# Wikinaut/agrep

Measured on NVIDIA H100. Metric: text_scan_throughput, higher is better.
Workload: dtype u32 bitwise

## Files before the change

agrep_b200/_lib.py:

```python
import ctypes as C
import os

HERE = os.path.dirname(os.path.abspath(__file__))
LIB_PATH = os.path.join(HERE, "libagrepb200.so")

AGB_MAXERR, AGB_MAXDELIM, AGB_MAXANCHOR = 8, 8, 24
WANT_COUNT, WANT_RECORDS, WANT_ORDINALS, WANT_LEVELS = 0, 1, 2, 4
PLAN_ALL, PLAN_ANCHORS = 0, 1
ENGINE_NAMES = {0: "bitap", 1: "asearch", 2: "asearch0", 3: "asearch1", 4: "sgrep_bm", 5: "regex"}
ENGINE_REGEX = 5
REGEX_MAXPOS = 63


class Options(C.Structure):
    _fields_ = [("k", C.c_int32), ("nocase", C.c_int32), ("wordbound", C.c_int32), ("wholeline", C.c_int32),
                ("inverse", C.c_int32), ("linenum", C.c_int32), ("ins_free", C.c_int32),
                ("cost_i", C.c_int32), ("cost_s", C.c_int32), ("cost_d", C.c_int32),
                ("bestmatch", C.c_int32), ("regex", C.c_int32), ("delim", C.c_char_p)]


class Desc(C.Structure):
    _fields_ = [("mask", C.c_uint64 * 256),
                ("init0", C.c_uint64), ("init1", C.c_uint64), ("noerr", C.c_uint64), ("endpos", C.c_uint64),
                ("dendpos", C.c_uint64), ("dmask", C.c_uint64), ("wildmask", C.c_uint64),
                ("reset", C.c_uint64 * (2 * AGB_MAXERR + 1)), ("start", C.c_uint64 * (2 * AGB_MAXERR + 1)),
                ("start_closes", C.c_int32), ("M", C.c_int32), ("L", C.c_int32),
                ("delim", C.c_uint8 * (2 * AGB_MAXDELIM + 2)),
                ("delim_kind", C.c_int32), ("k", C.c_int32), ("nrows", C.c_int32),
                ("cost_i", C.c_int32), ("cost_s", C.c_int32), ("cost_d", C.c_int32),
                ("engine", C.c_int32), ("and_mode", C.c_int32), ("inverse", C.c_int32),
                ("user_delim", C.c_int32), ("outtail", C.c_int32),
                ("plan", C.c_int32), ("n_anchors", C.c_int32), ("anchor_len", C.c_int32),
                ("anchor", C.c_uint32 * AGB_MAXANCHOR), ("anchor_fold", C.c_uint32), ("anchor_mask", C.c_uint32),
                ("refine", C.c_int32), ("pat_len", C.c_int32), ("anchor_off", C.c_int32 * AGB_MAXANCHOR),
                ("n_anchors3", C.c_int32), ("anchor3", C.c_uint32 * 4), ("anchor3_off", C.c_int32 * 4), ("adaptive", C.c_int32),
                ("delim_fold", C.c_uint8 * (2 * AGB_MAXDELIM + 2)), ("pad_", C.c_uint8 * 2)]


class Regex(C.Structure):
    _fields_ = [("follow", C.c_uint64 * (REGEX_MAXPOS + 1)), ("head", C.c_int32), ("tail", C.c_int32), ("pad", C.c_int32 * 2)]


class Record(C.Structure):
    _fields_ = [("begin", C.c_int64), ("end", C.c_int64), ("ordinal", C.c_int64), ("level", C.c_int32), ("pad", C.c_int32)]


class Result(C.Structure):
    _fields_ = [("n_matched", C.c_uint64), ("n_records", C.c_uint64), ("n_flagged", C.c_uint64),
                ("level_hist", C.c_uint64 * (AGB_MAXERR + 1)), ("ms_front", C.c_float), ("ms_records", C.c_float),
                ("n_closes", C.c_uint64), ("truncated", C.c_uint32), ("pad", C.c_uint32)]

# ... 82 lines not shown
```

agrep_b200/csrc/aux.cu:

```cuda
#include "automaton.cuh"
#include "corpus.h"

__global__ void __launch_bounds__(256) k_gram_sample(const uint8_t *text, uint64_t n_chunks, uint32_t nblk, uint32_t blk_chunks,
                                                    int ngram, const uint32_t *gram, const uint32_t *gmask, uint32_t fold, unsigned int *counts)
{
	__shared__ unsigned int s_cnt[128];
	if (threadIdx.x < 128) s_cnt[threadIdx.x] = 0;
	__syncthreads();
	const uint64_t t = (uint64_t)blockIdx.x * blockDim.x + threadIdx.x;
	const uint64_t b = t / blk_chunks, i = t % blk_chunks;
	if (b < nblk) {
		const uint64_t chunk = (n_chunks / nblk) * b + i;
		if (chunk + 2 < n_chunks) {
			const uint4 v = __ldg(reinterpret_cast<const uint4 *>(text) + chunk);
			const uint32_t x4 = __ldg(reinterpret_cast<const uint32_t *>(text) + (chunk + 1) * 4);
			const uint32_t x[5] = { v.x | fold, v.y | fold, v.z | fold, v.w | fold, x4 | fold };
			uint32_t wv[16];
#pragma unroll
			for (int w = 0; w < 4; w++) {
				wv[4 * w] = x[w]; wv[4 * w + 1] = __funnelshift_r(x[w], x[w + 1], 8);
				wv[4 * w + 2] = __funnelshift_r(x[w], x[w + 1], 16); wv[4 * w + 3] = __funnelshift_r(x[w], x[w + 1], 24);
			}
			for (int g = 0; g < ngram; g++) {
				const uint32_t G = gram[g], M = gmask[g];
				bool hit = false;
#pragma unroll
				for (int s = 0; s < 16; s++) hit = hit || ((wv[s] & M) == G);
				if (hit) atomicAdd(&s_cnt[g], 1u);
			}
		}
	}
	__syncthreads();
	if (threadIdx.x < ngram && s_cnt[threadIdx.x]) atomicAdd(&counts[threadIdx.x], s_cnt[threadIdx.x]);
}

__global__ void __launch_bounds__(256) k_bitmap_sample(const uint32_t *bitmap, uint64_t n_words, uint32_t stride, unsigned long long *out)
{
	unsigned long long c = 0;
	for (uint64_t i = ((uint64_t)blockIdx.x * blockDim.x + threadIdx.x) * stride; i < n_words; i += (uint64_t)gridDim.x * blockDim.x * stride)
		c += __popc(bitmap[i]);
	c = __reduce_add_sync(0xffffffffu, (uint32_t)c);
	if ((threadIdx.x & 31) == 0 && c) atomicAdd(out, c);
}

__global__ void __launch_bounds__(COMPACT_THREADS) k_compact_count(const uint32_t *bitmap, uint64_t n_words, uint32_t *block_counts, unsigned long long *totals)
{
	const uint64_t w0 = ((uint64_t)blockIdx.x * COMPACT_THREADS + threadIdx.x) * COMPACT_WPT;
	uint32_t c = 0;
// ... 361 lines not shown
```

agrep_b200/csrc/front.cu:

```cuda
#include "scan_internal.cuh"
#include "tma.cuh"


template <int NA, bool MASKED, bool POLY, int N3>
__device__ __forceinline__ uint32_t windows_test(uint32_t lo, uint32_t hi, const FrontParams &P, uint32_t acc)
{
	uint32_t w[4] = { lo, __funnelshift_r(lo, hi, 8), __funnelshift_r(lo, hi, 16), __funnelshift_r(lo, hi, 24) };
	if (POLY && N3 > 0) {
#pragma unroll
		for (int t = 0; t < 4; t++) {
			uint32_t r = (NA >= 2) ? __viaddmin_u32(w[t], P.coef[NA - 1], 0xFFFFFFFFu) : w[t] * P.one + P.coef[NA - 1];
#pragma unroll
			for (int i = NA - 2; i >= 0; i--) r = r * w[t] + P.coef[i];
			if (MASKED) r *= P.scale;
			uint32_t q;
			if (N3 == 1) q = w[t] * P.s256 + P.coef3[0];
			else {
				q = w[t] * P.one + P.coef3[N3 - 1];
#pragma unroll
				for (int i = N3 - 2; i >= 0; i--) q = q * w[t] + P.coef3[i];
				q *= P.s256;
			}
			acc = __vimin3_u32(acc, r, q);
		}
// ... 10 lines not shown
		}
		acc = __vimin3_u32(acc, f[0], f[1]);
		acc = __vimin3_u32(acc, f[2], f[3]);
	} else {
		if (MASKED) { w[0] &= P.amask; w[1] &= P.amask; w[2] &= P.amask; w[3] &= P.amask; }
#pragma unroll
		for (int a = 0; a < NA; a++) {
			uint32_t A = P.anchor[a];
			acc = __vimin3_u32(acc, w[0] - A, w[1] - A);
			acc = __vimin3_u32(acc, w[2] - A, w[3] - A);
		}
	}
	return acc;
}

template <int NA, bool MASKED, bool FOLD, bool POLY, bool FULL, bool COUNT, int N3>
__device__ __forceinline__ void front_chunks(const FrontParams &P, const uint8_t *st, uint32_t tid, uint32_t lane, uint32_t rem, uint32_t *bm, uint16_t *nlb)
{
#pragma unroll
	for (int c = 0; c < FRONT_CH; c++) {
		const uint32_t idx = c * FRONT_THREADS + tid;
		uint4 v = *reinterpret_cast<const uint4 *>(st + idx * 16);
		uint32_t x4 = *reinterpret_cast<const uint32_t *>(st + idx * 16 + 16);
		if (COUNT) {
			const uint32_t xs[4] = { v.x, v.y, v.z, v.w };
			uint32_t cn = 0;
#pragma unroll
			for (int w = 0; w < 4; w++) {
				const uint32_t t = (xs[w] | P.dfold4) ^ P.delim4;
				uint32_t z = ~(((t & 0x7F7F7F7Fu) + 0x7F7F7F7Fu) | t | 0x7F7F7F7Fu);
				if (!FULL) {
					const int64_t valid = ((int64_t)rem - (int64_t)idx) * 16 - (int64_t)(P.n_chunks * 16 - P.n) - 4 * w;
					if (valid <= 0) z = 0; else if (valid < 4) z &= (1u << (8 * (uint32_t)valid)) - 1u;
				}
				cn += __popc(z);
			}
			const uint32_t blk = __reduce_add_sync(0xffffffffu, cn);
			if (lane == 0 && (FULL || idx < rem)) nlb[c * (FRONT_THREADS / 32)] = (uint16_t)blk;
		}
		if (FOLD) { v.x |= P.fold; v.y |= P.fold; v.z |= P.fold; v.w |= P.fold; x4 |= P.fold; }
		uint32_t acc = 0xffffffffu;
		acc = windows_test<NA, MASKED, POLY, N3>(v.x, v.y, P, acc);
		acc = windows_test<NA, MASKED, POLY, N3>(v.y, v.z, P, acc);
		acc = windows_test<NA, MASKED, POLY, N3>(v.z, v.w, P, acc);
		acc = windows_test<NA, MASKED, POLY, N3>(v.w, x4, P, acc);
		if (FULL) {
			const uint32_t word = __ballot_sync(0xffffffffu, acc == 0);
			if (lane == 0) bm[c * (FRONT_THREADS / 32)] = word;
		} else {
			const bool flag = (idx < rem) && (acc == 0 || idx + 2 >= rem);
			const uint32_t word = __ballot_sync(0xffffffffu, flag);
			if (lane == 0 && idx < rem) bm[c * (FRONT_THREADS / 32)] = word;
		}
	}
}

template <int NA, bool MASKED, bool FOLD, bool POLY, bool COUNT, int N3>
__global__ void __launch_bounds__(FRONT_THREADS, FRONT_CTAS_PER_SM)
k_front(const FrontParams P)
{
	extern __shared__ __align__(128) uint8_t s_ring[];
	__shared__ uint64_t s_bar[FRONT_NST];
	const uint32_t tid = threadIdx.x, lane = tid & 31;
	if (tid == 0) {
		for (int i = 0; i < FRONT_NST; i++) mbar_init(&s_bar[i], 1);
		asm volatile("fence.mbarrier_init.release.cluster;" ::: "memory");
	}
	__syncthreads();
	auto issue = [&](uint64_t it) {
		const uint64_t sg = P.stage_begin + blockIdx.x + it * gridDim.x;
		if (sg >= P.stage_end) return;
		const uint32_t slot = (uint32_t)(it % FRONT_NST);
// ... 2 lines not shown
		mbar_expect_tx(&s_bar[slot], bytes);
		bulk_g2s(s_ring + slot * FRONT_SLOT_BYTES, P.text + off, bytes, &s_bar[slot]);
	};
	if (tid == 0) for (int i = 0; i < FRONT_NST; i++) issue(i);
	const uint32_t warp_in_cta = tid >> 5;
	for (uint32_t it = 0;; it++) {
		const uint64_t sg = P.stage_begin + blockIdx.x + (uint64_t)it * gridDim.x;
		if (sg >= P.stage_end) break;
		const uint32_t slot = it % FRONT_NST;
		mbar_wait(&s_bar[slot], (it / FRONT_NST) & 1u);
		const uint8_t *st = s_ring + slot * FRONT_SLOT_BYTES;
		const uint64_t left = P.n_chunks - sg * FRONT_STAGE_CHUNKS;
		const uint32_t rem = left > 0xFFFF0000ull ? 0xFFFF0000u : (uint32_t)left;
		uint32_t *bm = P.bitmap + sg * FRONT_WORDS_PER_STAGE + warp_in_cta;
		const bool full = left >= FRONT_STAGE_CHUNKS + 2;
		uint16_t *nlb = COUNT ? P.nl_blocks + sg * FRONT_WORDS_PER_STAGE + warp_in_cta : nullptr;
		if (full) front_chunks<NA, MASKED, FOLD, POLY, true, COUNT, N3>(P, st, tid, lane, rem, bm, nlb);
		else front_chunks<NA, MASKED, FOLD, POLY, false, COUNT, N3>(P, st, tid, lane, rem, bm, nlb);
		__syncthreads();
		if (tid == 0) issue((uint64_t)it + FRONT_NST);
	}
}

template <int NA, bool MASKED, bool FOLD, bool POLY, bool COUNT, int N3>
static void launch_front_cnt(const FrontParams &P, unsigned grid, cudaStream_t st)
{
	static bool configured[64] = {false};
	int dev = 0; cudaGetDevice(&dev);
	if (!configured[dev & 63]) {
		cudaFuncSetAttribute(k_front<NA, MASKED, FOLD, POLY, COUNT, N3>, cudaFuncAttributeMaxDynamicSharedMemorySize, FRONT_SMEM);
		configured[dev & 63] = true;
	}
	k_front<NA, MASKED, FOLD, POLY, COUNT, N3><<<grid, FRONT_THREADS, FRONT_SMEM, st>>>(P);
}
template <int NA, bool MASKED, bool FOLD, bool POLY, int N3>
static void launch_front_one(const FrontParams &P, unsigned grid, cudaStream_t st)
{
	if (P.nl_blocks) launch_front_cnt<NA, MASKED, FOLD, POLY, true, N3>(P, grid, st);
	else launch_front_cnt<NA, MASKED, FOLD, POLY, false, N3>(P, grid, st);
}
template <int NA, bool POLY>
static void launch_front_na(const FrontParams &P, bool masked, bool fold, unsigned grid, cudaStream_t st)
{
	if (masked) { if (fold) launch_front_one<NA, true, true, POLY, 0>(P, grid, st); else launch_front_one<NA, true, false, POLY, 0>(P, grid, st); }
	else        { if (fold) launch_front_one<NA, false, true, POLY, 0>(P, grid, st); else launch_front_one<NA, false, false, POLY, 0>(P, grid, st); }
}
template <int NA>
static void launch_front_mixed(const FrontParams &P, bool fold, unsigned grid, cudaStream_t st)
// ... 247 lines not shown
	F.stage_end = (word_end + FRONT_WORDS_PER_STAGE - 1) / FRONT_WORDS_PER_STAGE;
	F.fold = d.anchor_fold; F.amask = d.anchor_mask;
	F.nl_blocks = count_delims ? W.ord_blocks : nullptr; F.dfold4 = d.delim_fold[0] * 0x01010101u; F.delim4 = (d.delim[0] | d.delim_fold[0]) * 0x01010101u;
	const uint64_t stages = F.stage_end - F.stage_begin;
	unsigned grid = (unsigned)std::min<uint64_t>(stages, (uint64_t)W.sm_count * FRONT_CTAS_PER_SM);
	if (!grid) grid = 1;
	bool masked = d.anchor_mask != 0xFFFFFFFFu, fold = d.anchor_fold != 0;
	int na = 0;
	for (int i = 0; i < d.n_anchors; i++) {
		bool dup = false;
		for (int j = 0; j < na; j++) if (F.anchor[j] == d.anchor[i]) dup = true;
		if (!dup) F.anchor[na++] = d.anchor[i];
	}
	F.one = 1; F.scale = 1; F.s256 = 256;
	for (int i = d.anchor_len; i < 4; i++) F.scale <<= 8;
	bool poly = poly_setup(F.anchor, na, 8 * d.anchor_len, F.coef);
	if (d.n_anchors3 > 0) {
		int n3 = 0; uint32_t a3[4];
		for (int i = 0; i < d.n_anchors3; i++) {
			bool dup = false;
			for (int j = 0; j < n3; j++) if (a3[j] == d.anchor3[i]) dup = true;
			if (!dup) a3[n3++] = d.anchor3[i];
		}
		uint32_t c3[AGB_MAXANCHOR];
		const bool poly3 = poly_setup(a3, n3, 24, c3);
		if (!(poly && poly3)) { snprintf(g_err, sizeof g_err, "internal: mixed anchor plan without a polynomial form"); return AGB_ERR_ARG; }
		F.n3 = n3;
		for (int i = 0; i < n3; i++) F.coef3[i] = c3[i];
		if (n3 == 1) F.coef3[0] = 0u - 256u * a3[0];
		switch (na) {
// ... 46 lines not shown
```

agrep_b200/csrc/pattern.c:

```c
#include "agrep_b200.h"
#include "pattern_internal.h"
#include <stdio.h>
#include <stdlib.h>
#include <string.h>

#define WIDTH 64
#define FAIL(...) do { if (err && errlen) snprintf(err, errlen, __VA_ARGS__); return AGB_ERR_PATTERN; } while (0)

enum { S_HYPHEN = 129, S_NOCARE = 130, S_NNLINE = 131, S_WORDB = 133, S_LPAREN = 134, S_RPAREN = 135,
       S_LRANGE = 136, S_RRANGE = 137, S_LANGLE = 138, S_RANGLE = 139, S_NOT = 140, S_WILD = 141,
       S_ORSYM = 142, S_ORPAT = 143, S_ANDPAT = 144, S_STAR = 145 };

typedef struct {
	uint64_t cls[4];
	int is_sep;
	int prot;
	int wild;
	int lit;
	int part;
} pos_t;

typedef struct {
	pos_t p[WIDTH + 4];
	int n;
// ... 733 lines not shown
	return AGB_OK;
}

int agb_pattern_from_desc(const agb_desc *d, agb_pattern **out, char *err, size_t errlen)
{
	agb_pattern *p; int rc;
	if (err && errlen) err[0] = 0;
	if (!d || !out) return AGB_ERR_ARG;
	p = (agb_pattern *)calloc(1, sizeof *p);
	if (!p) return AGB_ERR_NOMEM;
	p->d = *d;
	if (p->d.plan != AGB_PLAN_ANCHORS || p->d.n_anchors < 1 || p->d.n_anchors > AGB_MAXANCHOR || p->d.anchor_len < 2 || p->d.anchor_len > 4) {
		p->d.plan = AGB_PLAN_ALL; p->d.n_anchors = 0; p->d.refine = 0;
	}
	if (p->d.n_anchors3 < 0 || p->d.n_anchors3 > 2 || p->d.plan != AGB_PLAN_ANCHORS) p->d.n_anchors3 = 0;
	rc = agbi_derive(&p->d, err, errlen);
	if (rc) { free(p); *out = NULL; return rc; }
	*out = p;
	return AGB_OK;
}

void agb_pattern_free(agb_pattern *p) { free(p); }
const agb_desc *agb_pattern_desc(const agb_pattern *p) { return p ? &p->d : NULL; }

void agb_fill_ordinals(const agb_pattern *p, const void *h_text, uint64_t n, agb_record *records, uint64_t n_records)
{
	const agb_desc *d = &p->d; const unsigned char *t = (const unsigned char *)h_text;
	const int L = d->L; uint64_t i = 0; long long j = 0, run = 0, q, taken = -(1ll << 60); unsigned char fd[2 * AGB_MAXDELIM + 2]; int z, head = 1;
	if (!n_records) return;
	folded_delim(d, fd);
// ... 30 lines not shown
```

agrep_b200/csrc/scan.cu:

```cuda
#include "scan_internal.cuh"
#include "corpus.h"
#include <unistd.h>
#include <fcntl.h>
#include <sys/stat.h>
#include <mutex>
#include <thread>

thread_local char g_err[512];
std::atomic<uint64_t> g_launches{0};

extern "C" const char *agb_last_error(void) { return g_err; }
extern "C" const char *agb_version(void) { return "agrep-b200 0.1 (sm_90a)"; }
extern "C" uint64_t agb_kernel_launches(void) { return g_launches.load(); }
static void win_release(int dev);
extern "C" void agb_shutdown(void)
{
	int cur = 0; cudaGetDevice(&cur);
	for (int dev = 0; dev < 64; dev++) {
		win_release(dev);
		std::lock_guard<std::mutex> lk(g_ws_mu[dev]);
		Workspace &W = g_ws[dev];
		if (!W.totals && !W.bitmap && !W.h2d_text) continue;
		if (cudaSetDevice(dev) != cudaSuccess) { cudaGetLastError(); continue; }
		cudaDeviceSynchronize();
// ... 210 lines not shown
	res->n_closes = (want & AGB_WANT_ORDINALS) ? W.h_totals[13] + (uint64_t)W.ord_virt : 0;
	return AGB_OK;
}

static int ordinals_prepare_blocks(const agb_desc &d, Workspace &W, uint64_t n, cudaStream_t st)
{
	int rc = ordinals_reserve(d, W, n); if (rc) return rc;
	const uint64_t n_words = ((n + 15) / 16 + 31) / 32;
	if (W.ord_blocks_cap > n_words) CUDA_TRY(cudaMemsetAsync(W.ord_blocks + n_words, 0, (W.ord_blocks_cap - n_words) * sizeof(uint16_t), st));
	return AGB_OK;
}

#define PLAN_MIN_BYTES   (256ull << 20)
#define PLAN_SAMPLE_BLK  64
#define PLAN_BLK_CHUNKS  4096
static int adaptive_plan(const agb_desc &d, Workspace &W, const void *d_text, uint64_t n, cudaStream_t st, agb_desc *out)
{
	*out = d;
	if (!d.adaptive || !front_usable(d) || !d.refine || d.n_anchors3 || n < PLAN_MIN_BYTES || d.pat_len < 4 || d.pat_len > 60) return AGB_OK;
	const int need = d.k + 1;
	if (need > 9) return AGB_OK;
	uint64_t key = 1469598103934665603ull;
	{
		const unsigned char *b = (const unsigned char *)&d;
		for (size_t i = 0; i < sizeof d; i++) { key ^= b[i]; key *= 1099511628211ull; }
		key ^= (uint64_t)(uintptr_t)d_text; key *= 1099511628211ull; key ^= n; key *= 1099511628211ull;
	}
	if (W.plan_valid && W.plan_key == key) { *out = W.plan_desc; return AGB_OK; }
	int lit[64]; bool pair_any = false;
	for (int j = 0; j < d.pat_len; j++) {
		const uint64_t bit = 1ull << (d.M - (d.L + 2 + j));
		int cnt = 0, c0 = -1, c1 = -1;
		for (int c = 0; c < 256; c++) if (d.mask[c] & bit) { if (cnt == 0) c0 = c; else if (cnt == 1) c1 = c; cnt++; }
		lit[j] = -1;
		if (cnt == 1 && c0 != '\n' && c0 < 0x80) lit[j] = c0;
		else if (cnt == 2 && (c0 ^ c1) == 0x20 && c1 < 0x80) { lit[j] = c0 | 0x20; pair_any = true; }
	}
	const uint32_t fold = pair_any ? 0x20202020u : 0u;
	struct Gram { int s, len; uint32_t v, m; double cost; };
	Gram g[128]; int ng = 0;
	for (int len = 4; len >= 3; len--)
		for (int s = 0; s + len <= d.pat_len && ng < 120; s++) {
			bool ok = true; uint32_t v = 0;
			for (int t = 0; t < len; t++) { if (lit[s + t] < 0) ok = false; else v |= (uint32_t)(lit[s + t] | (fold & 0x20)) << (8 * t); }
			if (!ok) continue;
			g[ng].s = s; g[ng].len = len; g[ng].v = v; g[ng].m = len == 4 ? 0xFFFFFFFFu : 0x00FFFFFFu; g[ng].cost = 0; ng++;
		}
	if (ng < need) return AGB_OK;
	if (!W.d_gram) { CUDA_TRY(cudaMalloc(&W.d_gram, 3 * 128 * sizeof(uint32_t))); CUDA_TRY(cudaMallocHost(&W.h_gram, 3 * 128 * sizeof(uint32_t))); }
	for (int i = 0; i < 128; i++) { W.h_gram[i] = i < ng ? g[i].v : 0; W.h_gram[128 + i] = i < ng ? g[i].m : 0; W.h_gram[256 + i] = 0; }
	CUDA_TRY(cudaMemcpyAsync(W.d_gram, W.h_gram, 3 * 128 * sizeof(uint32_t), cudaMemcpyHostToDevice, st));
	const uint64_t n_chunks = (n + 15) / 16;
	const uint64_t threads = (uint64_t)PLAN_SAMPLE_BLK * PLAN_BLK_CHUNKS;
	k_gram_sample<<<(unsigned)((threads + 255) / 256), 256, 0, st>>>((const uint8_t *)d_text, n_chunks, PLAN_SAMPLE_BLK, PLAN_BLK_CHUNKS,
	                                                                 ng, W.d_gram, W.d_gram + 128, fold, W.d_gram + 256);
	g_launches++;
	CUDA_TRY(cudaGetLastError());
	CUDA_TRY(cudaMemcpyAsync(W.h_gram + 256, W.d_gram + 256, 128 * sizeof(uint32_t), cudaMemcpyDeviceToHost, st));
	CUDA_TRY(cudaStreamSynchronize(st));
	for (int i = 0; i < ng; i++) g[i].cost = (double)W.h_gram[256 + i] / (double)threads;
	const char *mp = getenv("AGB_PLAN_MIXED");
	const double INF = 1e30, MIXED = mp ? atof(mp) : 0.03;
	static double f[66][10][3]; static int from[66][10][3];
	for (int p = 0; p <= d.pat_len; p++) for (int j = 0; j <= need; j++) for (int t = 0; t < 3; t++) { f[p][j][t] = INF; from[p][j][t] = -2; }
	f[0][0][0] = 0;
	for (int p = 0; p < d.pat_len; p++)
		for (int j = 0; j <= need; j++) for (int t = 0; t < 3; t++) {
			if (f[p][j][t] >= INF) continue;
			if (f[p][j][t] < f[p + 1][j][t]) { f[p + 1][j][t] = f[p][j][t]; from[p + 1][j][t] = -1; }
			if (j == need) continue;
			for (int i = 0; i < ng; i++) if (g[i].s == p) {
				const int t2 = t + (g[i].len == 3), p2 = p + g[i].len;
				if (t2 > 2) continue;
				if (f[p][j][t] + g[i].cost < f[p2][j + 1][t2]) { f[p2][j + 1][t2] = f[p][j][t] + g[i].cost; from[p2][j + 1][t2] = i; }
			}
		}
	int best_t = -1; double best = INF;
	for (int t = 0; t < 3; t++) {
		if (need - t < 1 || need - t > (t ? 7 : 9)) continue;
		const double c = f[d.pat_len][need][t] + (t ? MIXED : 0);
		if (c < best) { best = c; best_t = t; }
	}
	double cur = 0;
	for (int a = 0; a < d.n_anchors; a++) { double r = 1.0; for (int i = 0; i < ng; i++) if (g[i].len == d.anchor_len && g[i].s == d.anchor_off[a]) r = g[i].cost; cur += r; }
	if (best_t < 0 || !(best < 0.85 * cur)) { W.plan_key = key; W.plan_valid = true; W.plan_desc = d; return AGB_OK; }
	agb_desc nd = d;
	nd.n_anchors = 0; nd.n_anchors3 = 0; nd.anchor_len = 4; nd.anchor_mask = 0xFFFFFFFFu; nd.anchor_fold = fold;
	{
		int p = d.pat_len, j = need, t = best_t;
		while (p > 0 && j >= 0) {
			const int fr = from[p][j][t];
			if (fr == -1) { p--; continue; }
			if (fr < 0) break;
			if (g[fr].len == 4) { nd.anchor[nd.n_anchors] = g[fr].v; nd.anchor_off[nd.n_anchors] = g[fr].s; nd.n_anchors++; }
			else { nd.anchor3[nd.n_anchors3] = g[fr].v; nd.anchor3_off[nd.n_anchors3] = g[fr].s; nd.n_anchors3++; }
			p -= g[fr].len; j--; t -= (g[fr].len == 3);
		}
	}
	bool ok = nd.n_anchors + nd.n_anchors3 == need && nd.n_anchors >= 1;
	uint32_t tmp[AGB_MAXANCHOR];
	if (ok) ok = poly_setup(nd.anchor, nd.n_anchors, 32, tmp);
	if (ok && nd.n_anchors3) ok = poly_setup(nd.anchor3, nd.n_anchors3, 24, tmp);
	for (int a = 0; a < nd.n_anchors && ok; a++) {
		for (int b = 0; b < a; b++) if (nd.anchor[a] == nd.anchor[b]) ok = false;
		for (int b = 0; b < nd.n_anchors3; b++) if ((nd.anchor[a] & 0x00FFFFFFu) == nd.anchor3[b]) ok = false;
	}
	for (int a = 0; a < nd.n_anchors3 && ok; a++) for (int b = 0; b < a; b++) if (nd.anchor3[a] == nd.anchor3[b]) ok = false;
	W.plan_key = key; W.plan_valid = true; W.plan_desc = ok ? nd : d;
	*out = W.plan_desc;
	if (getenv("AGB_DEBUG_PLAN")) {
		fprintf(stderr, "agb plan: static rate %.4f -> %s rate %.4f:", cur, ok ? "chosen" : "rejected", best);
		for (int a = 0; a < nd.n_anchors; a++) fprintf(stderr, " [%.4s]@%d", (const char *)&nd.anchor[a], nd.anchor_off[a]);
		for (int a = 0; a < nd.n_anchors3; a++) fprintf(stderr, " [%.3s]@%d", (const char *)&nd.anchor3[a], nd.anchor3_off[a]);
		fprintf(stderr, "\n");
	}
	return AGB_OK;
}

int shard_aux_enqueue(const agb_desc &d, Workspace &W, const uint8_t *text, uint64_t n, const ShardInfo *sh, bool ordinals, cudaStream_t st);

static int stages_after_front(const agb_desc &d, Workspace &W, const void *d_text, uint64_t n, bool use_front, bool count_in_front,
                              int want, int want_level, agb_record *d_records, uint64_t capacity, cudaStream_t st, agb_result *res,
                              const ShardInfo *sh = nullptr)
{
	int rc;
	const uint64_t n_chunks = (n + 15) / 16;
	if (use_front && refine_cannot_thin(d)) { bool dense = false; rc = front_is_dense(W, n, st, &dense); if (rc) return rc; if (dense) use_front = false; }
	bool refined = false;
	if (use_front) { rc = refine_launch(d, W, d_text, n, st, &refined); if (rc) return rc; }
	for (int attempt = 0; ; attempt++) {
// ... 34 lines not shown
		agb_result r;
		int rc = scan_device_impl(pos, d_text, n, AGB_WANT_COUNT | AGB_WANT_ORDINALS, -1, nullptr, 0, st, &r, nullptr); if (rc) return rc;
		unsigned char last = 0;
		CUDA_TRY(cudaMemcpyAsync(&last, (const uint8_t *)d_text + n - 1, 1, cudaMemcpyDeviceToHost, st));
		CUDA_TRY(cudaStreamSynchronize(st));
		const uint64_t records = r.n_closes - 2 + (last != '\n' ? 1 : 0);
		if (r.n_closes < 2 || r.n_matched > records) { snprintf(g_err, sizeof g_err, "internal: complement count out of range"); return AGB_ERR_CUDA; }
		*res = r;
		res->n_matched = records - r.n_matched; res->n_closes = 0; res->n_records = 0;
		return AGB_OK;
	}
	std::lock_guard<std::mutex> lk(g_ws_mu[dev]);
	Workspace &W = g_ws[dev];
	int rc = ws_prepare(W, n); if (rc) return rc;
	agb_desc planned;
	rc = adaptive_plan(d_in, W, d_text, n, st, &planned); if (rc) return rc;
	const agb_desc &d = planned;
	if (want == AGB_WANT_COUNT && !sh && n >= (1u << 20) && exact_count_usable(d)) {
		CUDA_TRY(cudaMemsetAsync(W.totals, 0, 16 * sizeof(unsigned long long), st));
		CUDA_TRY(cudaEventRecord(W.e0, st));
		rc = exact_count_launch(d, W, d_text, n, st); if (rc) return rc;
		CUDA_TRY(cudaEventRecord(W.e1, st));
		CUDA_TRY(cudaEventRecord(W.e2, st));
		rc = fetch_result(W, want, capacity, false, st, res); if (rc) return rc;
		res->n_flagged = 0;
		CUDA_TRY(cudaEventElapsedTime(&res->ms_front, W.e0, W.e1));
		res->ms_records = 0;
		return AGB_OK;
	}
	rc = ws_upload_desc(W, d, st); if (rc) return rc;
	rc = regex_prepare(W, d, rx, st); if (rc) return rc;
// ... 603 lines not shown
```

agrep_b200/csrc/scan_internal.cuh:

```cuda
#ifndef AGB_SCAN_INTERNAL_CUH
#define AGB_SCAN_INTERNAL_CUH
#include "agrep_b200.h"
#include "pattern_internal.h"
#include <cuda_runtime.h>
#include <stdint.h>
#include <stdio.h>
#include <string.h>
#include <stdlib.h>
#include <atomic>
#include <algorithm>

extern thread_local char g_err[512];
extern std::atomic<uint64_t> g_launches;

#define CUDA_TRY(x) do { cudaError_t e_ = (x); if (e_ != cudaSuccess) { \
	snprintf(g_err, sizeof g_err, "%s failed: %s (%s:%d)", #x, cudaGetErrorString(e_), __FILE__, __LINE__); \
	return AGB_ERR_CUDA; } } while (0)

#define FRONT_THREADS 256
#define FRONT_CH      4
#define FRONT_STAGE_CHUNKS (FRONT_THREADS * FRONT_CH)
#define FRONT_STAGE_BYTES  (FRONT_STAGE_CHUNKS * 16)
#define FRONT_SLOT_BYTES   (FRONT_STAGE_BYTES + 16)
#define FRONT_NST     2
// ... 140 lines not shown
int  exact_count_launch(const agb_desc &d, Workspace &W, const void *d_text, uint64_t n, cudaStream_t st);
bool poly_setup(const uint32_t *a, int na, int bits, uint32_t *coef);
int  front_launch(const agb_desc &d, Workspace &W, const void *d_text, uint64_t n, uint64_t word_begin, uint64_t word_end, bool slack16, cudaStream_t st, bool count_delims = false);
int  refine_launch(const agb_desc &d, Workspace &W, const void *d_text, uint64_t n, cudaStream_t st, bool *ran);
unsigned refine_grid(const Workspace &W, uint64_t n);
int  compact_ranges_launch(Workspace &W, uint64_t n, cudaStream_t st);
#define REFINE_MAX_RANGES 16384
int  launch_records(const agb_desc &d, const RecParams &P, unsigned grid, cudaStream_t st);
int  launch_dense(const agb_desc &d, const RecParams &P, unsigned grid, cudaStream_t st);
int  launch_records_list(const agb_desc &d, const RecParams &P, unsigned grid, cudaStream_t st);
int  launch_slices(const agb_desc &d, const RecParams &P, unsigned grid, cudaStream_t st);
bool slices_usable(const agb_desc &d);
int  launch_regex(const agb_desc &d, const RecParams &P, unsigned grid, cudaStream_t st);
size_t regex_tables(const agb_desc &d, const agb_regex &rx, uint64_t *out);
__global__ void k_gram_sample(const uint8_t *text, uint64_t n_chunks, uint32_t nblk, uint32_t blk_chunks,
                              int ngram, const uint32_t *gram, const uint32_t *gmask, uint32_t fold, unsigned int *counts);
__global__ void k_compact_count(const uint32_t *bitmap, uint64_t n_words, uint32_t *block_counts, unsigned long long *totals);
__global__ void k_compact_write(const uint32_t *bitmap, uint64_t n_words, const uint64_t *block_offsets, uint64_t *cand, uint64_t cand_cap);
__global__ void k_scan_tiles(const uint32_t *counts, uint64_t *offsets, uint64_t n_tiles, unsigned long long *total);
__global__ void k_scan_partial(const uint32_t *counts, uint64_t n, uint32_t *block_sums, const unsigned long long *n_dev);
__global__ void k_scan_apply(const uint32_t *counts, uint64_t n, const uint64_t *block_offsets, uint64_t *offsets, const unsigned long long *n_dev);
int  front_is_dense(Workspace &W, uint64_t n, cudaStream_t st, bool *dense);
int  ordinals_launch(const agb_desc &d, Workspace &W, const void *d_text, uint64_t n, agb_record *d_records, uint64_t capacity, cudaStream_t st, bool blocks_counted = false);
int  ordinals_reserve(const agb_desc &d, Workspace &W, uint64_t n);
#endif
```

include/agrep_b200.h:

```cpp
#ifndef AGREP_B200_H
#define AGREP_B200_H
#include <stdint.h>
#include <stddef.h>

#ifdef __cplusplus
extern "C" {
#endif

#define AGB_MAXERR    8
#define AGB_MAXDELIM  8
#define AGB_MAXANCHOR 24

enum {
	AGB_OK = 0,
	AGB_ERR_PATTERN = -1,
	AGB_ERR_CUDA = -2,
	AGB_ERR_ARG = -3,
	AGB_ERR_NOMEM = -4
};

typedef struct agb_options {
	int32_t k;
	int32_t nocase;
	int32_t wordbound;
// ... 30 lines not shown
	int32_t  nrows;
	int32_t  cost_i, cost_s, cost_d;
	int32_t  engine, and_mode, inverse, user_delim, outtail;
	int32_t  plan;
	int32_t  n_anchors, anchor_len;
	uint32_t anchor[AGB_MAXANCHOR];
	uint32_t anchor_fold;
	uint32_t anchor_mask;
	int32_t  refine, pat_len;
	int32_t  anchor_off[AGB_MAXANCHOR];
	int32_t  n_anchors3;
	uint32_t anchor3[4];
	int32_t  anchor3_off[4];
	int32_t  adaptive;
	uint8_t  delim_fold[2 * AGB_MAXDELIM + 2];
	uint8_t  pad_[2];
} agb_desc;

typedef struct agb_pattern agb_pattern;

#define AGB_REGEX_MAXPOS 63
typedef struct agb_regex {
	uint64_t follow[AGB_REGEX_MAXPOS + 1];
	int32_t  head, tail;
	int32_t  pad[2];
} agb_regex;

typedef struct agb_record {
	int64_t begin;
	int64_t end;
	int64_t ordinal;
// ... 95 lines not shown
```

Before: 2081.

## Add pair-of-pieces anchor filter plan chosen by adaptive sampling

Adds a new candidate-filter plan that splits the pattern into k+2 disjoint literal pieces and flags a chunk only when at least two distinct pieces occur within it or the adjacent chunk. The sampler now also measures the rate of this pair condition, and the planner picks it when that rate is well below the k+1 anchor plan's rate and delimiter counting for ordinals is not needed. The goal is fewer false-positive candidates reaching the costlier verification stage. In exchange the front kernel does per-piece presence checks with warp shuffles, and the sampling kernel does a second window load on hits.

Measured after the change: 2311, median of 6. 11.1% higher.

```diff
diff --git a/agrep_b200/_lib.py b/agrep_b200/_lib.py
--- a/agrep_b200/_lib.py
+++ b/agrep_b200/_lib.py
@@ -34,7 +34,7 @@
                 ("anchor", C.c_uint32 * AGB_MAXANCHOR), ("anchor_fold", C.c_uint32), ("anchor_mask", C.c_uint32),
                 ("refine", C.c_int32), ("pat_len", C.c_int32), ("anchor_off", C.c_int32 * AGB_MAXANCHOR),
                 ("n_anchors3", C.c_int32), ("anchor3", C.c_uint32 * 4), ("anchor3_off", C.c_int32 * 4), ("adaptive", C.c_int32),
-                ("delim_fold", C.c_uint8 * (2 * AGB_MAXDELIM + 2)), ("pad_", C.c_uint8 * 2)]
+                ("delim_fold", C.c_uint8 * (2 * AGB_MAXDELIM + 2)), ("pair_plan", C.c_uint8), ("pad_", C.c_uint8)]
 
 
 class Regex(C.Structure):
diff --git a/agrep_b200/csrc/aux.cu b/agrep_b200/csrc/aux.cu
--- a/agrep_b200/csrc/aux.cu
+++ b/agrep_b200/csrc/aux.cu
@@ -1,8 +1,27 @@
 #include "automaton.cuh"
 #include "corpus.h"
 
+__device__ __forceinline__ void sample_windows(const uint8_t *text, uint64_t chunk, uint32_t fold, uint32_t (&wv)[16])
+{
+	const uint4 v = __ldg(reinterpret_cast<const uint4 *>(text) + chunk);
+	const uint32_t x4 = __ldg(reinterpret_cast<const uint32_t *>(text) + (chunk + 1) * 4);
+	const uint32_t x[5] = { v.x | fold, v.y | fold, v.z | fold, v.w | fold, x4 | fold };
+#pragma unroll
+	for (int w = 0; w < 4; w++) {
+		wv[4 * w] = x[w]; wv[4 * w + 1] = __funnelshift_r(x[w], x[w + 1], 8);
+		wv[4 * w + 2] = __funnelshift_r(x[w], x[w + 1], 16); wv[4 * w + 3] = __funnelshift_r(x[w], x[w + 1], 24);
+	}
+}
+__device__ __forceinline__ bool sample_hit(const uint32_t (&wv)[16], uint32_t G, uint32_t M)
+{
+	bool hit = false;
+#pragma unroll
+	for (int s = 0; s < 16; s++) hit = hit || ((wv[s] & M) == G);
+	return hit;
+}
 __global__ void __launch_bounds__(256) k_gram_sample(const uint8_t *text, uint64_t n_chunks, uint32_t nblk, uint32_t blk_chunks,
-                                                    int ngram, const uint32_t *gram, const uint32_t *gmask, uint32_t fold, unsigned int *counts)
+                                                    int ngram, const uint32_t *gram, const uint32_t *gmask, uint32_t fold, unsigned int *counts,
+                                                    int pair_first, int n_pair)
 {
 	__shared__ unsigned int s_cnt[128];
 	if (threadIdx.x < 128) s_cnt[threadIdx.x] = 0;
@@ -12,26 +31,24 @@
 	if (b < nblk) {
 		const uint64_t chunk = (n_chunks / nblk) * b + i;
 		if (chunk + 2 < n_chunks) {
-			const uint4 v = __ldg(reinterpret_cast<const uint4 *>(text) + chunk);
-			const uint32_t x4 = __ldg(reinterpret_cast<const uint32_t *>(text) + (chunk + 1) * 4);
-			const uint32_t x[5] = { v.x | fold, v.y | fold, v.z | fold, v.w | fold, x4 | fold };
 			uint32_t wv[16];
-#pragma unroll
-			for (int w = 0; w < 4; w++) {
-				wv[4 * w] = x[w]; wv[4 * w + 1] = __funnelshift_r(x[w], x[w + 1], 8);
-				wv[4 * w + 2] = __funnelshift_r(x[w], x[w + 1], 16); wv[4 * w + 3] = __funnelshift_r(x[w], x[w + 1], 24);
+			sample_windows(text, chunk, fold, wv);
+			uint32_t here = 0;
+			for (int g = 0; g < ngram; g++) {
+				if (!sample_hit(wv, gram[g], gmask[g])) continue;
+				if (g < 127) atomicAdd(&s_cnt[g], 1u);
+				if (g >= pair_first && g < pair_first + n_pair) here |= 1u << (g - pair_first);
 			}
-			for (int g = 0; g < ngram; g++) {
-				const uint32_t G = gram[g], M = gmask[g];
-				bool hit = false;
-#pragma unroll
-				for (int s = 0; s < 16; s++) hit = hit || ((wv[s] & M) == G);
-				if (hit) atomicAdd(&s_cnt[g], 1u);
+			if (here) {
+				uint32_t next = 0;
+				sample_windows(text, chunk + 1, fold, wv);
+				for (int p = 0; p < n_pair; p++) if (sample_hit(wv, gram[pair_first + p], gmask[pair_first + p])) next |= 1u << p;
+				if (__popc(here | next) >= 2) atomicAdd(&s_cnt[127], 1u);
 			}
 		}
 	}
 	__syncthreads();
-	if (threadIdx.x < ngram && s_cnt[threadIdx.x]) atomicAdd(&counts[threadIdx.x], s_cnt[threadIdx.x]);
+	if (threadIdx.x < 128 && s_cnt[threadIdx.x]) atomicAdd(&counts[threadIdx.x], s_cnt[threadIdx.x]);
 }
 
 __global__ void __launch_bounds__(256) k_bitmap_sample(const uint32_t *bitmap, uint64_t n_words, uint32_t stride, unsigned long long *out)
diff --git a/agrep_b200/csrc/front.cu b/agrep_b200/csrc/front.cu
--- a/agrep_b200/csrc/front.cu
+++ b/agrep_b200/csrc/front.cu
@@ -48,6 +48,24 @@
 	return acc;
 }
 
+template <bool FULL>
+__device__ __forceinline__ uint32_t chunk_delims(const FrontParams &P, const uint4 v, uint32_t idx, uint32_t rem)
+{
+	const uint32_t xs[4] = { v.x, v.y, v.z, v.w };
+	uint32_t cn = 0;
+#pragma unroll
+	for (int w = 0; w < 4; w++) {
+		const uint32_t t = (xs[w] | P.dfold4) ^ P.delim4;
+		uint32_t z = ~(((t & 0x7F7F7F7Fu) + 0x7F7F7F7Fu) | t | 0x7F7F7F7Fu);
+		if (!FULL) {
+			const int64_t valid = ((int64_t)rem - (int64_t)idx) * 16 - (int64_t)(P.n_chunks * 16 - P.n) - 4 * w;
+			if (valid <= 0) z = 0; else if (valid < 4) z &= (1u << (8 * (uint32_t)valid)) - 1u;
+		}
+		cn += __popc(z);
+	}
+	return cn;
+}
+
 template <int NA, bool MASKED, bool FOLD, bool POLY, bool FULL, bool COUNT, int N3>
 __device__ __forceinline__ void front_chunks(const FrontParams &P, const uint8_t *st, uint32_t tid, uint32_t lane, uint32_t rem, uint32_t *bm, uint16_t *nlb)
 {
@@ -57,19 +75,7 @@
 		uint4 v = *reinterpret_cast<const uint4 *>(st + idx * 16);
 		uint32_t x4 = *reinterpret_cast<const uint32_t *>(st + idx * 16 + 16);
 		if (COUNT) {
-			const uint32_t xs[4] = { v.x, v.y, v.z, v.w };
-			uint32_t cn = 0;
-#pragma unroll
-			for (int w = 0; w < 4; w++) {
-				const uint32_t t = (xs[w] | P.dfold4) ^ P.delim4;
-				uint32_t z = ~(((t & 0x7F7F7F7Fu) + 0x7F7F7F7Fu) | t | 0x7F7F7F7Fu);
-				if (!FULL) {
-					const int64_t valid = ((int64_t)rem - (int64_t)idx) * 16 - (int64_t)(P.n_chunks * 16 - P.n) - 4 * w;
-					if (valid <= 0) z = 0; else if (valid < 4) z &= (1u << (8 * (uint32_t)valid)) - 1u;
-				}
-				cn += __popc(z);
-			}
-			const uint32_t blk = __reduce_add_sync(0xffffffffu, cn);
+			const uint32_t blk = __reduce_add_sync(0xffffffffu, chunk_delims<FULL>(P, v, idx, rem));
 			if (lane == 0 && (FULL || idx < rem)) nlb[c * (FRONT_THREADS / 32)] = (uint16_t)blk;
 		}
 		if (FOLD) { v.x |= P.fold; v.y |= P.fold; v.z |= P.fold; v.w |= P.fold; x4 |= P.fold; }
@@ -89,7 +95,68 @@
 	}
 }
 
-template <int NA, bool MASKED, bool FOLD, bool POLY, bool COUNT, int N3>
+
+__device__ __forceinline__ uint32_t imad(uint32_t a, uint32_t b, uint32_t c)
+{
+	uint32_t r; asm("mad.lo.u32 %0, %1, %2, %3;" : "=r"(r) : "r"(a), "r"(b), "r"(c)); return r;
+}
+
+template <int NP>
+__device__ __forceinline__ uint32_t piece_bits(const uint32_t (&x)[5], const FrontParams &P)
+{
+	uint32_t acc[NP];
+#pragma unroll
+	for (int i = 0; i < NP; i++) acc[i] = 1u;
+#pragma unroll
+	for (int w = 0; w < 4; w++) {
+		const uint32_t wv[4] = { x[w], __funnelshift_r(x[w], x[w + 1], 8), __funnelshift_r(x[w], x[w + 1], 16), __funnelshift_r(x[w], x[w + 1], 24) };
+#pragma unroll
+		for (int i = 0; i < NP; i++) {
+			acc[i] = __vimin3_u32(acc[i], imad(wv[0], P.scale, P.coef[i]), imad(wv[1], P.scale, P.coef[i]));
+			acc[i] = __vimin3_u32(acc[i], imad(wv[2], P.scale, P.coef[i]), imad(wv[3], P.scale, P.coef[i]));
+		}
+	}
+	uint32_t absent = 0;
+#pragma unroll
+	for (int i = 0; i < NP; i++) absent |= acc[i] << i;
+	return absent ^ ((1u << NP) - 1u);
+}
+
+template <int NP, bool FOLD, bool FULL, bool COUNT>
+__device__ __forceinline__ void pair_chunks(const FrontParams &P, const uint8_t *st, uint32_t wid, uint32_t lane, uint32_t rem, uint32_t *bm, uint16_t *nlb)
+{
+	uint32_t pres[FRONT_CH];
+#pragma unroll
+	for (int c = 0; c < FRONT_CH; c++) {
+		const uint32_t idx = (wid * FRONT_CH + c) * 32 + lane;
+		const uint4 v = *reinterpret_cast<const uint4 *>(st + idx * 16);
+		const uint32_t x4 = *reinterpret_cast<const uint32_t *>(st + idx * 16 + 16);
+		if (COUNT) {
+			const uint32_t blk = __reduce_add_sync(0xffffffffu, chunk_delims<FULL>(P, v, idx, rem));
+			if (lane == 0 && (FULL || idx < rem)) nlb[c] = (uint16_t)blk;
+		}
+		const uint32_t f = FOLD ? P.fold : 0u;
+		const uint32_t x[5] = { v.x | f, v.y | f, v.z | f, v.w | f, x4 | f };
+		pres[c] = piece_bits<NP>(x, P);
+	}
+#pragma unroll
+	for (int c = 0; c < FRONT_CH; c++) {
+		const uint32_t idx = (wid * FRONT_CH + c) * 32 + lane;
+		const uint32_t give = (lane == 0 && c + 1 < FRONT_CH) ? pres[c + 1] : pres[c];
+		uint32_t next = __shfl_sync(0xffffffffu, give, (lane + 1) & 31);
+		if (c + 1 == FRONT_CH && lane == 31) next = ~0u;
+		const bool pair = pres[c] != 0 && __popc(pres[c] | next) >= 2;
+		if (FULL) {
+			const uint32_t word = __ballot_sync(0xffffffffu, pair);
+			if (lane == 0) bm[c] = word;
+		} else {
+			const uint32_t word = __ballot_sync(0xffffffffu, (idx < rem) && (pair || idx + 2 >= rem));
+			if (lane == 0 && idx < rem) bm[c] = word;
+		}
+	}
+}
+
+template <int NA, bool MASKED, bool FOLD, bool POLY, bool COUNT, int N3, int NP = 0>
 __global__ void __launch_bounds__(FRONT_THREADS, FRONT_CTAS_PER_SM)
 k_front(const FrontParams P)
 {
@@ -122,24 +189,37 @@
 		const uint32_t rem = left > 0xFFFF0000ull ? 0xFFFF0000u : (uint32_t)left;
 		uint32_t *bm = P.bitmap + sg * FRONT_WORDS_PER_STAGE + warp_in_cta;
 		const bool full = left >= FRONT_STAGE_CHUNKS + 2;
-		uint16_t *nlb = COUNT ? P.nl_blocks + sg * FRONT_WORDS_PER_STAGE + warp_in_cta : nullptr;
-		if (full) front_chunks<NA, MASKED, FOLD, POLY, true, COUNT, N3>(P, st, tid, lane, rem, bm, nlb);
-		else front_chunks<NA, MASKED, FOLD, POLY, false, COUNT, N3>(P, st, tid, lane, rem, bm, nlb);
+		if constexpr (NP > 0) {
+			uint32_t *bmp = P.bitmap + sg * FRONT_WORDS_PER_STAGE + warp_in_cta * FRONT_CH;
+			uint16_t *nlp = COUNT ? P.nl_blocks + sg * FRONT_WORDS_PER_STAGE + warp_in_cta * FRONT_CH : nullptr;
+			if (full) pair_chunks<NP, FOLD, true, COUNT>(P, st, warp_in_cta, lane, rem, bmp, nlp);
+			else pair_chunks<NP, FOLD, false, COUNT>(P, st, warp_in_cta, lane, rem, bmp, nlp);
+		} else {
+			uint16_t *nlb = COUNT ? P.nl_blocks + sg * FRONT_WORDS_PER_STAGE + warp_in_cta : nullptr;
+			if (full) front_chunks<NA, MASKED, FOLD, POLY, true, COUNT, N3>(P, st, tid, lane, rem, bm, nlb);
+			else front_chunks<NA, MASKED, FOLD, POLY, false, COUNT, N3>(P, st, tid, lane, rem, bm, nlb);
+		}
 		__syncthreads();
 		if (tid == 0) issue((uint64_t)it + FRONT_NST);
 	}
 }
 
-template <int NA, bool MASKED, bool FOLD, bool POLY, bool COUNT, int N3>
+template <int NA, bool MASKED, bool FOLD, bool POLY, bool COUNT, int N3, int NP = 0>
 static void launch_front_cnt(const FrontParams &P, unsigned grid, cudaStream_t st)
 {
 	static bool configured[64] = {false};
 	int dev = 0; cudaGetDevice(&dev);
 	if (!configured[dev & 63]) {
-		cudaFuncSetAttribute(k_front<NA, MASKED, FOLD, POLY, COUNT, N3>, cudaFuncAttributeMaxDynamicSharedMemorySize, FRONT_SMEM);
+		cudaFuncSetAttribute(k_front<NA, MASKED, FOLD, POLY, COUNT, N3, NP>, cudaFuncAttributeMaxDynamicSharedMemorySize, FRONT_SMEM);
 		configured[dev & 63] = true;
 	}
-	k_front<NA, MASKED, FOLD, POLY, COUNT, N3><<<grid, FRONT_THREADS, FRONT_SMEM, st>>>(P);
+	k_front<NA, MASKED, FOLD, POLY, COUNT, N3, NP><<<grid, FRONT_THREADS, FRONT_SMEM, st>>>(P);
+}
+template <int NP>
+static void launch_front_pairs(const FrontParams &P, bool fold, unsigned grid, cudaStream_t st)
+{
+	if (P.nl_blocks) { if (fold) launch_front_cnt<0, false, true, true, true, 0, NP>(P, grid, st); else launch_front_cnt<0, false, false, true, true, 0, NP>(P, grid, st); }
+	else             { if (fold) launch_front_cnt<0, false, true, true, false, 0, NP>(P, grid, st); else launch_front_cnt<0, false, false, true, false, 0, NP>(P, grid, st); }
 }
 template <int NA, bool MASKED, bool FOLD, bool POLY, int N3>
 static void launch_front_one(const FrontParams &P, unsigned grid, cudaStream_t st)
@@ -417,6 +497,18 @@
 	}
 	F.one = 1; F.scale = 1; F.s256 = 256;
 	for (int i = d.anchor_len; i < 4; i++) F.scale <<= 8;
+	if (d.pair_plan) {
+		if (na != d.n_anchors || na < 2 || na > 4 || d.anchor_len < 3) { snprintf(g_err, sizeof g_err, "internal: pair plan with %d pieces", d.n_anchors); return AGB_ERR_ARG; }
+		for (int i = 0; i < na; i++) F.coef[i] = 0u - F.anchor[i] * F.scale;
+		switch (na) {
+		case 2: launch_front_pairs<2>(F, fold, grid, st); break;
+		case 3: launch_front_pairs<3>(F, fold, grid, st); break;
+		default: launch_front_pairs<4>(F, fold, grid, st); break;
+		}
+		g_launches++;
+		CUDA_TRY(cudaGetLastError());
+		return AGB_OK;
+	}
 	bool poly = poly_setup(F.anchor, na, 8 * d.anchor_len, F.coef);
 	if (d.n_anchors3 > 0) {
 		int n3 = 0; uint32_t a3[4];
diff --git a/agrep_b200/csrc/pattern.c b/agrep_b200/csrc/pattern.c
--- a/agrep_b200/csrc/pattern.c
+++ b/agrep_b200/csrc/pattern.c
@@ -771,6 +771,7 @@
 		p->d.plan = AGB_PLAN_ALL; p->d.n_anchors = 0; p->d.refine = 0;
 	}
 	if (p->d.n_anchors3 < 0 || p->d.n_anchors3 > 2 || p->d.plan != AGB_PLAN_ANCHORS) p->d.n_anchors3 = 0;
+	p->d.pair_plan = 0;
 	rc = agbi_derive(&p->d, err, errlen);
 	if (rc) { free(p); *out = NULL; return rc; }
 	*out = p;
diff --git a/agrep_b200/csrc/scan.cu b/agrep_b200/csrc/scan.cu
--- a/agrep_b200/csrc/scan.cu
+++ b/agrep_b200/csrc/scan.cu
@@ -248,17 +248,45 @@
 #define PLAN_MIN_BYTES   (256ull << 20)
 #define PLAN_SAMPLE_BLK  64
 #define PLAN_BLK_CHUNKS  4096
-static int adaptive_plan(const agb_desc &d, Workspace &W, const void *d_text, uint64_t n, cudaStream_t st, agb_desc *out)
+#define PAIR_REACH       16
+
+static int pair_pieces(const int *lit, int pat_len, int k, uint32_t fold, uint32_t *val, int *off, int *len_out)
+{
+	const int np = k + 2;
+	if (k < 0 || np > 4) return 0;
+	for (int len = 4; len >= 3; len--)
+		for (int s0 = 0; s0 + np * len <= pat_len; s0++) {
+			int got = 0;
+			for (int p = s0; p + len <= pat_len && got < np; ) {
+				bool ok = true; uint32_t v = 0;
+				for (int t = 0; t < len; t++) { if (lit[p + t] < 0) ok = false; else v |= (uint32_t)(lit[p + t] | (fold & 0x20)) << (8 * t); }
+				if (!ok) { p++; continue; }
+				val[got] = v; off[got] = p; got++; p += len;
+			}
+			if (got < np || off[0] != s0 || off[np - 1] - off[0] + k > PAIR_REACH) continue;
+			bool distinct = true;
+			for (int a = 0; a < np; a++) for (int b = 0; b < a; b++) if (val[a] == val[b]) distinct = false;
+			if (!distinct) continue;
+			*len_out = len;
+			return np;
+		}
+	return 0;
+}
+
+static int adaptive_plan(const agb_desc &d, Workspace &W, const void *d_text, uint64_t n, bool count_delims, cudaStream_t st, agb_desc *out)
 {
 	*out = d;
 	if (!d.adaptive || !front_usable(d) || !d.refine || d.n_anchors3 || n < PLAN_MIN_BYTES || d.pat_len < 4 || d.pat_len > 60) return AGB_OK;
 	const int need = d.k + 1;
 	if (need > 9) return AGB_OK;
+	const char *pp = getenv("AGB_PLAN_PAIRS");
+	const int pairs_env = (pp && *pp) ? atoi(pp) : -1;
 	uint64_t key = 1469598103934665603ull;
 	{
 		const unsigned char *b = (const unsigned char *)&d;
 		for (size_t i = 0; i < sizeof d; i++) { key ^= b[i]; key *= 1099511628211ull; }
 		key ^= (uint64_t)(uintptr_t)d_text; key *= 1099511628211ull; key ^= n; key *= 1099511628211ull;
+		key ^= (uint64_t)(pairs_env + 2) * 2 + (count_delims ? 1 : 0); key *= 1099511628211ull;
 	}
 	if (W.plan_valid && W.plan_key == key) { *out = W.plan_desc; return AGB_OK; }
 	int lit[64]; bool pair_any = false;
@@ -280,19 +308,27 @@
 			if (!ok) continue;
 			g[ng].s = s; g[ng].len = len; g[ng].v = v; g[ng].m = len == 4 ? 0xFFFFFFFFu : 0x00FFFFFFu; g[ng].cost = 0; ng++;
 		}
-	if (ng < need) return AGB_OK;
+	uint32_t pv[4]; int poff[4], plen = 0;
+	const int n_pair = pairs_env != 0 ? pair_pieces(lit, d.pat_len, d.k, fold, pv, poff, &plen) : 0;
+	if (ng < need && !n_pair) return AGB_OK;
 	if (!W.d_gram) { CUDA_TRY(cudaMalloc(&W.d_gram, 3 * 128 * sizeof(uint32_t))); CUDA_TRY(cudaMallocHost(&W.h_gram, 3 * 128 * sizeof(uint32_t))); }
-	for (int i = 0; i < 128; i++) { W.h_gram[i] = i < ng ? g[i].v : 0; W.h_gram[128 + i] = i < ng ? g[i].m : 0; W.h_gram[256 + i] = 0; }
+	for (int i = 0; i < 128; i++) {
+		const bool gi = i < ng, pi = i >= ng && i < ng + n_pair;
+		W.h_gram[i] = gi ? g[i].v : pi ? pv[i - ng] : 0;
+		W.h_gram[128 + i] = gi ? g[i].m : pi ? (plen == 4 ? 0xFFFFFFFFu : 0x00FFFFFFu) : 0;
+		W.h_gram[256 + i] = 0;
+	}
 	CUDA_TRY(cudaMemcpyAsync(W.d_gram, W.h_gram, 3 * 128 * sizeof(uint32_t), cudaMemcpyHostToDevice, st));
 	const uint64_t n_chunks = (n + 15) / 16;
 	const uint64_t threads = (uint64_t)PLAN_SAMPLE_BLK * PLAN_BLK_CHUNKS;
 	k_gram_sample<<<(unsigned)((threads + 255) / 256), 256, 0, st>>>((const uint8_t *)d_text, n_chunks, PLAN_SAMPLE_BLK, PLAN_BLK_CHUNKS,
-	                                                                 ng, W.d_gram, W.d_gram + 128, fold, W.d_gram + 256);
+	                                                                 ng + n_pair, W.d_gram, W.d_gram + 128, fold, W.d_gram + 256, ng, n_pair);
 	g_launches++;
 	CUDA_TRY(cudaGetLastError());
 	CUDA_TRY(cudaMemcpyAsync(W.h_gram + 256, W.d_gram + 256, 128 * sizeof(uint32_t), cudaMemcpyDeviceToHost, st));
 	CUDA_TRY(cudaStreamSynchronize(st));
 	for (int i = 0; i < ng; i++) g[i].cost = (double)W.h_gram[256 + i] / (double)threads;
+	const double pair_rate = (double)W.h_gram[256 + 127] / (double)threads;
 	const char *mp = getenv("AGB_PLAN_MIXED");
 	const double INF = 1e30, MIXED = mp ? atof(mp) : 0.03;
 	static double f[66][10][3]; static int from[66][10][3];
@@ -317,37 +353,56 @@
 	}
 	double cur = 0;
 	for (int a = 0; a < d.n_anchors; a++) { double r = 1.0; for (int i = 0; i < ng; i++) if (g[i].len == d.anchor_len && g[i].s == d.anchor_off[a]) r = g[i].cost; cur += r; }
-	if (best_t < 0 || !(best < 0.85 * cur)) { W.plan_key = key; W.plan_valid = true; W.plan_desc = d; return AGB_OK; }
-	agb_desc nd = d;
-	nd.n_anchors = 0; nd.n_anchors3 = 0; nd.anchor_len = 4; nd.anchor_mask = 0xFFFFFFFFu; nd.anchor_fold = fold;
-	{
-		int p = d.pat_len, j = need, t = best_t;
-		while (p > 0 && j >= 0) {
-			const int fr = from[p][j][t];
-			if (fr == -1) { p--; continue; }
-			if (fr < 0) break;
-			if (g[fr].len == 4) { nd.anchor[nd.n_anchors] = g[fr].v; nd.anchor_off[nd.n_anchors] = g[fr].s; nd.n_anchors++; }
-			else { nd.anchor3[nd.n_anchors3] = g[fr].v; nd.anchor3_off[nd.n_anchors3] = g[fr].s; nd.n_anchors3++; }
-			p -= g[fr].len; j--; t -= (g[fr].len == 3);
-		}
-	}
-	bool ok = nd.n_anchors + nd.n_anchors3 == need && nd.n_anchors >= 1;
-	uint32_t tmp[AGB_MAXANCHOR];
-	if (ok) ok = poly_setup(nd.anchor, nd.n_anchors, 32, tmp);
-	if (ok && nd.n_anchors3) ok = poly_setup(nd.anchor3, nd.n_anchors3, 24, tmp);
-	for (int a = 0; a < nd.n_anchors && ok; a++) {
-		for (int b = 0; b < a; b++) if (nd.anchor[a] == nd.anchor[b]) ok = false;
-		for (int b = 0; b < nd.n_anchors3; b++) if ((nd.anchor[a] & 0x00FFFFFFu) == nd.anchor3[b]) ok = false;
-	}
-	for (int a = 0; a < nd.n_anchors3 && ok; a++) for (int b = 0; b < a; b++) if (nd.anchor3[a] == nd.anchor3[b]) ok = false;
-	W.plan_key = key; W.plan_valid = true; W.plan_desc = ok ? nd : d;
-	*out = W.plan_desc;
-	if (getenv("AGB_DEBUG_PLAN")) {
-		fprintf(stderr, "agb plan: static rate %.4f -> %s rate %.4f:", cur, ok ? "chosen" : "rejected", best);
-		for (int a = 0; a < nd.n_anchors; a++) fprintf(stderr, " [%.4s]@%d", (const char *)&nd.anchor[a], nd.anchor_off[a]);
-		for (int a = 0; a < nd.n_anchors3; a++) fprintf(stderr, " [%.3s]@%d", (const char *)&nd.anchor3[a], nd.anchor3_off[a]);
-		fprintf(stderr, "\n");
-	}
+	agb_desc plan = d;
+	double rate = cur;
+	if (best_t >= 0 && best < 0.85 * cur) {
+		agb_desc nd = d;
+		nd.n_anchors = 0; nd.n_anchors3 = 0; nd.anchor_len = 4; nd.anchor_mask = 0xFFFFFFFFu; nd.anchor_fold = fold;
+		{
+			int p = d.pat_len, j = need, t = best_t;
+			while (p > 0 && j >= 0) {
+				const int fr = from[p][j][t];
+				if (fr == -1) { p--; continue; }
+				if (fr < 0) break;
+				if (g[fr].len == 4) { nd.anchor[nd.n_anchors] = g[fr].v; nd.anchor_off[nd.n_anchors] = g[fr].s; nd.n_anchors++; }
+				else { nd.anchor3[nd.n_anchors3] = g[fr].v; nd.anchor3_off[nd.n_anchors3] = g[fr].s; nd.n_anchors3++; }
+				p -= g[fr].len; j--; t -= (g[fr].len == 3);
+			}
+		}
+		bool ok = nd.n_anchors + nd.n_anchors3 == need && nd.n_anchors >= 1;
+		uint32_t tmp[AGB_MAXANCHOR];
+		if (ok) ok = poly_setup(nd.anchor, nd.n_anchors, 32, tmp);
+		if (ok && nd.n_anchors3) ok = poly_setup(nd.anchor3, nd.n_anchors3, 24, tmp);
+		for (int a = 0; a < nd.n_anchors && ok; a++) {
+			for (int b = 0; b < a; b++) if (nd.anchor[a] == nd.anchor[b]) ok = false;
+			for (int b = 0; b < nd.n_anchors3; b++) if ((nd.anchor[a] & 0x00FFFFFFu) == nd.anchor3[b]) ok = false;
+		}
+		for (int a = 0; a < nd.n_anchors3 && ok; a++) for (int b = 0; b < a; b++) if (nd.anchor3[a] == nd.anchor3[b]) ok = false;
+		if (ok) { plan = nd; rate = best; }
+		if (getenv("AGB_DEBUG_PLAN")) {
+			fprintf(stderr, "agb plan: static rate %.4f -> %s rate %.4f:", cur, ok ? "chosen" : "rejected", best);
+			for (int a = 0; a < nd.n_anchors; a++) fprintf(stderr, " [%.4s]@%d", (const char *)&nd.anchor[a], nd.anchor_off[a]);
+			for (int a = 0; a < nd.n_anchors3; a++) fprintf(stderr, " [%.3s]@%d", (const char *)&nd.anchor3[a], nd.anchor3_off[a]);
+			fprintf(stderr, "\n");
+		}
+	}
+	if (n_pair) {
+		const bool take = pairs_env == 1 || (!count_delims && pair_rate < 0.85 * rate);
+		if (take) {
+			agb_desc pd = d;
+			pd.pair_plan = 1; pd.n_anchors = n_pair; pd.n_anchors3 = 0; pd.anchor_len = plen;
+			pd.anchor_mask = plen == 4 ? 0xFFFFFFFFu : 0x00FFFFFFu; pd.anchor_fold = fold;
+			for (int i = 0; i < n_pair; i++) { pd.anchor[i] = pv[i]; pd.anchor_off[i] = poff[i]; }
+			plan = pd;
+		}
+		if (getenv("AGB_DEBUG_PLAN")) {
+			fprintf(stderr, "agb plan: k+1 rate %.4f, pair rate %.4f -> pair plan %s:", rate, pair_rate, take ? "chosen" : "not chosen");
+			for (int i = 0; i < n_pair; i++) fprintf(stderr, " [%.*s]@%d", plen, (const char *)&pv[i], poff[i]);
+			fprintf(stderr, "\n");
+		}
+	}
+	W.plan_key = key; W.plan_valid = true; W.plan_desc = plan;
+	*out = plan;
 	return AGB_OK;
 }
 
@@ -412,7 +467,7 @@
 	Workspace &W = g_ws[dev];
 	int rc = ws_prepare(W, n); if (rc) return rc;
 	agb_desc planned;
-	rc = adaptive_plan(d_in, W, d_text, n, st, &planned); if (rc) return rc;
+	rc = adaptive_plan(d_in, W, d_text, n, (want & AGB_WANT_ORDINALS) && d_in.L == 1, st, &planned); if (rc) return rc;
 	const agb_desc &d = planned;
 	if (want == AGB_WANT_COUNT && !sh && n >= (1u << 20) && exact_count_usable(d)) {
 		CUDA_TRY(cudaMemsetAsync(W.totals, 0, 16 * sizeof(unsigned long long), st));
diff --git a/agrep_b200/csrc/scan_internal.cuh b/agrep_b200/csrc/scan_internal.cuh
--- a/agrep_b200/csrc/scan_internal.cuh
+++ b/agrep_b200/csrc/scan_internal.cuh
@@ -178,7 +178,8 @@
 int  launch_regex(const agb_desc &d, const RecParams &P, unsigned grid, cudaStream_t st);
 size_t regex_tables(const agb_desc &d, const agb_regex &rx, uint64_t *out);
 __global__ void k_gram_sample(const uint8_t *text, uint64_t n_chunks, uint32_t nblk, uint32_t blk_chunks,
-                              int ngram, const uint32_t *gram, const uint32_t *gmask, uint32_t fold, unsigned int *counts);
+                              int ngram, const uint32_t *gram, const uint32_t *gmask, uint32_t fold, unsigned int *counts,
+                              int pair_first, int n_pair);
 __global__ void k_compact_count(const uint32_t *bitmap, uint64_t n_words, uint32_t *block_counts, unsigned long long *totals);
 __global__ void k_compact_write(const uint32_t *bitmap, uint64_t n_words, const uint64_t *block_offsets, uint64_t *cand, uint64_t cand_cap);
 __global__ void k_scan_tiles(const uint32_t *counts, uint64_t *offsets, uint64_t n_tiles, unsigned long long *total);
diff --git a/include/agrep_b200.h b/include/agrep_b200.h
--- a/include/agrep_b200.h
+++ b/include/agrep_b200.h
@@ -68,7 +68,8 @@
 	int32_t  anchor3_off[4];
 	int32_t  adaptive;
 	uint8_t  delim_fold[2 * AGB_MAXDELIM + 2];
-	uint8_t  pad_[2];
+	uint8_t  pair_plan;
+	uint8_t  pad_[1];
 } agb_desc;
 
 typedef struct agb_pattern agb_pattern;
```
